# LANL-Bioinformatics/FaQCs

Hardware: AMD Instinct MI355X
Metric: M reads/sec (paired 2x150bp) (higher is better)
Workload: dtype u8; 1 GPU; synthetic 100M-pair 2x150bp Q33 reads resident in HBM per GPU, BWA_plus -q 5 --min_L 50, 1 step = 1 pass (trim_lds + counter all-reduce); pairs_per_gpu=100000000, read_len=150, terminal_n_supplied=True

## Files before the change

### faqcs_amd/csrc/faqcs_trim_common.h

```cpp
#pragma once
#include "faqcs_dev.h"

#include <stdlib.h>

static inline hipError_t ensure_dynamic_lds(const void *kernel, size_t bytes, unsigned long long &done)
{
    int dev = 0;
    hipError_t e = hipGetDevice(&dev);
    if (e != hipSuccess) return e;
    const unsigned long long bit = 1ull << (dev & 63);
    if (__atomic_load_n(&done, __ATOMIC_ACQUIRE) & bit) return hipSuccess;
    e = hipFuncSetAttribute(kernel, hipFuncAttributeMaxDynamicSharedMemorySize, (int)bytes);
    if (e == hipSuccess) __atomic_fetch_or(&done, bit, __ATOMIC_RELEASE);
    return e;
}

namespace {

template <int D> struct __attribute__((packed, aligned(1))) PackedBytes { uint32_t w[D]; };

__device__ __forceinline__ int med3i(int x, int lo, int hi) { return x < lo ? lo : (x > hi ? hi : x); }

template <int C> __device__ __forceinline__ uint32_t range_mask(int lo, int hi, int pbase)
{
// ... 246 lines not shown
    uint32_t *c = lane < FAQCS_NQ ? hrq + lane : hbq + (lane - FAQCS_NQ);
    if (in) { lds_add_u32_quiet(c, 1u); lds_add_u32_quiet(c, 1u); lds_add_u32_quiet(c, v); }
}
#endif

template <bool COMBINE = true>
__device__ __forceinline__ void chunk_epilogue_pre(const bool mine, const bool e_err, const uint32_t e_len, const int Vpre, const int lane, uint32_t *hlen,
                                                   uint32_t *hrq, uint32_t *hbqpre, const uint32_t *t_magic, FsAcc *defer)
{
        int qb_pre = 0;
        if (mine && e_len > 0 && Vpre > 0) qb_pre = e_len == 1 ? Vpre : (int)__umulhi((uint32_t)Vpre, t_magic[e_len]);
        qb_pre = qb_pre > 41 ? 41 : qb_pre;
        const bool act = mine && !e_err;
#ifdef FAQCS_LDS_DIAG_EPI_NOCONFLICT
        epi_diag_adds(act, e_len, hrq, hbqpre, lane);
#else
        const unsigned long long actm = COMBINE ? __ballot(act) : 0ull;
        if (!COMBINE) {
            if (act) {
                const uint32_t key = e_len | ((uint32_t)qb_pre << 16);
                const bool same = key == (uint32_t)__builtin_amdgcn_readfirstlane((int)key);
                const uint32_t cnt = (uint32_t)__builtin_popcountll(__ballot(same));
                if (same) {
                    if (lane == __ffsll((unsigned long long)__ballot(true)) - 1) {
                        lds_add_u32_quiet(hlen + e_len, cnt);
                        lds_add_u32_quiet(hrq + qb_pre, cnt);
                        if (e_len) lds_add_u32_quiet(hbqpre + qb_pre, cnt * e_len);
                    }
                } else {
                    lds_add_u32_quiet(hlen + e_len, 1u);
                    lds_add_u32_quiet(hrq + qb_pre, 1u);
                    if (e_len) lds_add_u32_quiet(hbqpre + qb_pre, e_len);
                }
            }
        } else if (actm != 0ull) {
            const uint32_t len0 = (uint32_t)__builtin_amdgcn_readlane((int)e_len, __builtin_ctzll(actm));
            const uint32_t cnt = wave_value_count(act, (uint32_t)qb_pre, lane);
            uint32_t bin = (uint32_t)lane;
            asm volatile("" : "+v"(bin));
            if (cnt) lds_add_u32_quiet(hrq + bin, cnt);
            len_hist_add(act, e_len, len0, 1u, hlen, lane);
            if (__ballot(act && e_len != len0) == 0ull) {
                if (cnt && len0) lds_add_u32_quiet(hbqpre + bin, cnt * len0);
            } else {
                peel_pairs(act && e_len != 0u, (uint32_t)qb_pre, e_len, nullptr, 0u, hbqpre, lane);
            }
        }
#endif
        const uint32_t one = 1u << 20;
        defer->tot += mine ? one | e_len : 0u;
}

template <int LPR>
__device__ __forceinline__ void chunk_epilogue(const ReadOutcome &o, const bool mine, const uint32_t my, const uint32_t v_len,
                                               const uint32_t v_hit, const int lane, uint32_t *hlen, uint32_t *hrq, uint32_t *hbqpre,
                                               uint32_t *hbqpost, uint32_t *lfs, const uint32_t *t_magic, uint2 *__restrict__ out,
                                               unsigned long long *__restrict__ rec_pre, unsigned long long *__restrict__ rec_post,
                                               const bool o_avgq_on, const uint32_t o_dbg, FsAcc *defer = nullptr, const bool wide_rt = false,
                                               const bool pre_done = false)
{
        const bool e_ret = (o.fl & FAQCS_F_VALID) != 0, e_err = (o.fl & FAQCS_F_ERR_QUALITY) != 0;
        const uint32_t e_len = v_len, e_n = o.an >> 16, e_filt = (o.fl & FAQCS_F_FILTER_MASK) >> FAQCS_F_FILTER_SHIFT;
        int qb_pre = 0, qb_post = 0;
        if (!defer && mine && e_len > 0 && o.Vpre > 0) qb_pre = e_len == 1 ? o.Vpre : (int)__umulhi((uint32_t)o.Vpre, t_magic[e_len]);
        if (e_ret && o.Vpost > 0) qb_post = e_n == 1 ? o.Vpost : (int)__umulhi((uint32_t)o.Vpost, t_magic[e_n]);
        qb_pre = qb_pre > 41 ? 41 : qb_pre;
        qb_post = qb_post > 41 ? 41 : qb_post;
        if (defer) {
            if (!pre_done) chunk_epilogue_pre<(LPR < 16)>(mine, e_err, e_len, o.Vpre, lane, hlen, hrq, hbqpre, t_magic, defer);
            const bool pact = mine && !e_err && e_ret;
#ifdef FAQCS_LDS_DIAG_EPI_NOCONFLICT
            epi_diag_adds(pact, e_n, hrq, hbqpost, lane);
#else
            const unsigned long long pm = LPR < 16 ? __ballot(pact) : 0ull;
            if (LPR >= 16) {
                if (pact) {
                    const uint32_t key = e_n | ((uint32_t)qb_post << 16);
                    const bool same = key == (uint32_t)__builtin_amdgcn_readfirstlane((int)key);
                    const uint32_t cnt = (uint32_t)__builtin_popcountll(__ballot(same));
                    if (same) {
                        if (lane == __ffsll((unsigned long long)__ballot(true)) - 1) {
                            lds_add_u32_quiet(hlen + e_n, cnt << 16);
                            lds_add_u32_quiet(hrq + qb_post, cnt << 16);
                            lds_add_u32_quiet(hbqpost + qb_post, cnt * e_n);
                        }
                    } else {
                        lds_add_u32_quiet(hlen + e_n, 0x10000u);
                        lds_add_u32_quiet(hrq + qb_post, 0x10000u);
                        lds_add_u32_quiet(hbqpost + qb_post, e_n);
                    }
                }
            } else if (pm != 0ull) {
                peel_pairs(pact, (uint32_t)qb_post, e_n, hrq, 0x10000u, hbqpost, lane);
                len_hist_add(pact, e_n, (uint32_t)__builtin_amdgcn_readlane((int)e_len, __builtin_ctzll(pm)), 0x10000u, hlen, lane);
            }
#endif
        } else if (!(o_dbg & 2u) && mine && !e_err) {
            atomicAdd(hlen + e_len, 1u);
            atomicAdd(hrq + qb_pre, 1u);
            if (e_len) atomicAdd(hbqpre + qb_pre, e_len);
            if (e_ret) {
                atomicAdd(hlen + e_n, 0x10000u);
                atomicAdd(hrq + qb_post, 0x10000u);
                atomicAdd(hbqpost + qb_post, e_n);
            }
        }
        if (mine) {
            const bool bad_base = v_hit == 0xffffu;
            out[my] = make_uint2(e_ret ? o.an : 0u, (o.fl & 0x3ffu) | (bad_base ? (uint32_t)FAQCS_F_ERR_BASE : (v_hit << 16)));
            const bool pre_on = !e_err, post_on = e_ret && !e_err;
            const unsigned long long pA = o.pAT & 0xffffu, pT = o.pAT >> 16, pC = o.pCG & 0xffffu, pG = o.pCG >> 16, pn = o.N & 0xffffu;
            const unsigned long long cA = o.cAT & 0xffffu, cT = o.cAT >> 16, cC = o.cCG & 0xffffu, cG = o.cCG >> 16, cn = o.N >> 16;
            if (LPR <= 16 && !wide_rt) {
                rec_pre[my] = pre_on ? (CR_VALID | e_len | (pA << 9) | (pT << 18) | (pC << 27) | (pG << 36) | (pn << 45)) : 0ull;
                rec_post[my] = post_on ? (CR_VALID | e_n | (cA << 9) | (cT << 18) | (cC << 27) | (cG << 36) | (cn << 45)) : 0ull;
            } else {
                reinterpret_cast<ulonglong2 *>(rec_pre)[my] =
                    pre_on ? make_ulonglong2(CR_VALID | e_len | (pA << 11) | (pT << 22) | (pC << 33), pG | (pn << 11)) : make_ulonglong2(0ull, 0ull);
                reinterpret_cast<ulonglong2 *>(rec_post)[my] =
                    post_on ? make_ulonglong2(CR_VALID | e_n | (cA << 11) | (cT << 22) | (cC << 33), cG | (cn << 11)) : make_ulonglong2(0ull, 0ull);
            }
        }
        const bool e_rlen = e_filt == FAQCS_FILT_LENGTH_PRE || e_filt == FAQCS_FILT_LENGTH_POST;
        const uint32_t one = 1u << 20;
        if (defer) {
            defer->trim += e_ret ? one | e_n : 0u;
            defer->len += e_rlen ? one | e_n : 0u;
            defer->qt += (o.fl & FAQCS_F_QUAL_TRIMMED) ? one | (o.fl >> 20) : 0u;
            const uint32_t m = one - 1u;
            const bool is_nn = (o.fl & FAQCS_F_POLY_N_SEEN) != 0, is_lc = e_filt == FAQCS_FILT_LOW_COMPLEXITY, is_avg = o_avgq_on && e_filt == FAQCS_FILT_AVG_Q;
            if (__any(is_nn)) { const uint32_t v = (uint32_t)wave_sum_i32((int)(is_nn ? one | e_n : 0u)); if (lane == 0) { lds_add_u32_quiet(&lfs[FAQCS_READ_NN], v >> 20); lds_add_u32_quiet(&lfs[FAQCS_BASE_NN], v & m); } }
            if (__any(is_lc)) { const uint32_t v = (uint32_t)wave_sum_i32((int)(is_lc ? one | e_n : 0u)); if (lane == 0) { lds_add_u32_quiet(&lfs[FAQCS_READ_LOW_COMPLEXITY], v >> 20); lds_add_u32_quiet(&lfs[FAQCS_BASE_LOW_COMPLEXITY], v & m); } }
            if (__any(is_avg)) { const uint32_t v = (uint32_t)wave_sum_i32((int)(is_avg ? one | e_n : 0u)); if (lane == 0) { lds_add_u32_quiet(&lfs[FAQCS_READ_AVG_Q], v >> 20); lds_add_u32_quiet(&lfs[FAQCS_BASE_AVG_Q], v & m); } }
            return;
        }
        const uint32_t s_tot = (uint32_t)wave_sum_i32((int)(mine ? one | e_len : 0u));
        const uint32_t s_trim = (uint32_t)wave_sum_i32((int)(e_ret ? one | e_n : 0u));
        const uint32_t s_len = (uint32_t)wave_sum_i32((int)(e_rlen ? one | e_n : 0u));
        const uint32_t s_nn = (uint32_t)wave_sum_i32((int)((o.fl & FAQCS_F_POLY_N_SEEN) ? one | e_n : 0u));
        const uint32_t s_qt = (uint32_t)wave_sum_i32((int)((o.fl & FAQCS_F_QUAL_TRIMMED) ? one | (o.fl >> 20) : 0u));
        const uint32_t s_lc = (uint32_t)wave_sum_i32((int)(e_filt == FAQCS_FILT_LOW_COMPLEXITY ? one | e_n : 0u));
        uint32_t s_avg = 0;
        if (o_avgq_on) s_avg = (uint32_t)wave_sum_i32((int)(e_filt == FAQCS_FILT_AVG_Q ? one | e_n : 0u));
        if (lane == 0) {
            const uint32_t m = one - 1u;
            if (s_tot) { atomicAdd(&lfs[FAQCS_TOTAL_COUNT], s_tot >> 20); atomicAdd(&lfs[FAQCS_TOTAL_NUMBER], s_tot >> 20); atomicAdd(&lfs[FAQCS_TOTAL_LENGTH], s_tot & m); }
            if (s_trim) { atomicAdd(&lfs[FAQCS_TOTAL_TRIMMED_NUMBER], s_trim >> 20); atomicAdd(&lfs[FAQCS_TOTAL_TRIMMED_LENGTH], s_trim & m); }
            if (s_len) { atomicAdd(&lfs[FAQCS_READ_LENGTH], s_len >> 20); atomicAdd(&lfs[FAQCS_BASE_LENGTH], s_len & m); }
            if (s_nn) { atomicAdd(&lfs[FAQCS_READ_NN], s_nn >> 20); atomicAdd(&lfs[FAQCS_BASE_NN], s_nn & m); }
            if (s_avg) { atomicAdd(&lfs[FAQCS_READ_AVG_Q], s_avg >> 20); atomicAdd(&lfs[FAQCS_BASE_AVG_Q], s_avg & m); }
            if (s_qt) { atomicAdd(&lfs[FAQCS_READ_QUAL_TRIM], s_qt >> 20); atomicAdd(&lfs[FAQCS_BASE_QUAL_TRIM], s_qt & m); }
            if (s_lc) { atomicAdd(&lfs[FAQCS_READ_LOW_COMPLEXITY], s_lc >> 20); atomicAdd(&lfs[FAQCS_BASE_LOW_COMPLEXITY], s_lc & m); }
        }
}

#ifdef __HIPCC__
__device__ __forceinline__ void comp_cell_add(uint32_t *tab, const uint32_t e, const uint32_t v, const int lane)
{
#ifdef FAQCS_DIAG_FOLD_NOCONFLICT
    constexpr uint32_t ND_ = (FAQCS_NCOMP_BIN * FAQCS_NCOMP_KIND + 1) / 2;
    uint32_t d = ((e >> 1) & ~63u) | (uint32_t)lane;
    d = d >= ND_ ? d - 64u : d;
    atomicAdd(&tab[d], v << (16 * (e & 1u)));
#else
    atomicAdd(&tab[e >> 1], v << (16 * (e & 1u)));
#endif
}
template <bool WIDE>
__device__ __forceinline__ void comp_fold_record(uint32_t *tab, const float *normt, const unsigned long long x, const unsigned long long y, const int lane)
{
    uint32_t nbin = 0xffffffffu;
    if (x & CR_VALID) {
        uint32_t len, cnt[5];
        if (WIDE) {
            len = (uint32_t)(x & 2047u);
// ... 97 lines not shown
```

### faqcs_amd/csrc/faqcs_trim_lds_kernel.hip

```cpp
#include "faqcs_trim_common.h"

#include <stdlib.h>
#include <type_traits>

#ifndef FAQCS_LDS_SUM_UNROLL
#define FAQCS_LDS_SUM_UNROLL 4
#endif
#ifndef FAQCS_LDS_SA_UNROLL
#define FAQCS_LDS_SA_UNROLL 2
#endif

namespace {

typedef uint32_t LdsPair2 __attribute__((ext_vector_type(2)));
typedef const __attribute__((address_space(3))) LdsPair2 *lds_u2c_ptr;
typedef __attribute__((address_space(3))) uint8_t *lds_u8_mut;
typedef const __attribute__((address_space(3))) uint8_t *lds_u8_ptr;
struct __attribute__((packed, aligned(1))) U32u { uint32_t w; };
typedef const __attribute__((address_space(3))) U32u *lds_u32u_ptr;

__device__ __forceinline__ uint32_t lds_ld(uint32_t byte_offset) { return *(lds_u32_ptr)(size_t)byte_offset; }
__device__ __forceinline__ uint32_t lds_ld_any(uint32_t byte_offset)
{
    const uint32_t a4 = byte_offset & ~3u;
// ... 601 lines not shown
                co += (uint32_t)__builtin_amdgcn_update_dpp(0, (int)co, 0x140, 0xf, 0xf, false);
            }
            tot_pe = turn ? pe : tot_pe; tot_po = turn ? po : tot_po; tot_ce = turn ? ce : tot_ce; tot_co = turn ? co : tot_co;
            if (WIDE) tot_pn = turn ? pn : tot_pn;
            }
            const uint32_t seam = e[C - 1].y & (uint32_t)__builtin_amdgcn_update_dpp(0, (int)e[0].y, 0x101, 0xf, 0xf, false) & 0x01000000u;
#ifdef FAQCS_LDS_DIAG_S_NO_NBLOCK
            const bool n_gate = false;
#else
            const bool n_gate = tq_lane + seam >= 0x02000000u || chk;
#endif
            if ((!EXT || P.max_poly_n == 2u) && __any(n_gate)) {
                uint32_t nb[D];
#pragma unroll
                for (int k = 0; k < D; ++k) {
                    const uint32_t orig = w[k] ^ (~((EXT && chk) ? 0u : inw[k]) & 0x88888888u);
                    const uint32_t x = (orig & inw[k]) ^ 0x4e4e4e4eu;
                    const uint32_t sx = (x & 0x7f7f7f7fu) + 0x7f7f7f7fu;
                    nb[k] = ~(sx | x) & 0x80808080u;
                }
                {
                    uint32_t hit = 0;
#pragma unroll
                    for (int k = 0; k < D; ++k) {
                        uint32_t here = nb[k];
                        if (4 * k + 4 > C) here &= low_bytes_(C - 4 * k);
                        const uint32_t next = k + 1 < D ? __builtin_amdgcn_alignbyte(nb[k + 1], nb[k], 1u) : (nb[k] >> 8);
                        hit |= here & next;
                    }
                    if (C % 4 == 0) hit |= (nb[D - 1] >> 24) & RW::next(nb[0] & 0x80u);
                    const bool rowhit = RW::all_or(hit) != 0u;
                    pairhit = turn ? rowhit : pairhit;
                }
            }
        }
    };
#define FAQCS_B_LOOP(I0, I1, CELLS)                                                                                   \
    {                                                                                                                 \
        _Pragma("unroll 1") for (int t = 0; t < TPR; ++t) {                                                          \
            if (base + (uint32_t)t >= n_reads) break;                       \
            const uint32_t a0_ = (uint32_t)__shfl((int)(I0), rowb + t), a1_ = (uint32_t)__shfl((int)(I1), rowb + t);   \
            RawB cur_;                                                                                                \
            load_b(a0_, a1_, cur_);                                                                                   \
            CELLS(cur_, a0_, a1_, t);                                                                                 \
        }                                                                                                             \
    }

#ifdef FAQCS_LDS_STAMPS
    unsigned long long st_acc[10] = {0, 0, 0, 0, 0, 0, 0, 0, 0, 0}, st_prev = 0, st_flush = 0, st_spill = 0;
#define FAQCS_STAMP(i) { const unsigned long long now_ = __builtin_amdgcn_s_memtime(); st_acc[i] += now_ - st_prev; st_prev = now_; }
#else
#define FAQCS_STAMP(i)
#endif
    uint32_t p_off = 0, p_end = 0, p_tn = 0;
    auto fetch_offsets = [&](const uint32_t chunk_) {
        if (chunk_ != NO_CHUNK) {
            const uint32_t lim_ = umin_(chunk_ * RPC + RPC, n_reads), my_ = owner ? chunk_ * RPC + ridx : lim_;
            p_off = off[my_ < lim_ ? my_ : lim_];
            p_end = off[my_ < lim_ ? my_ + 1 : lim_];
            if (tn_flags) p_tn = (uint32_t)tn_flags[my_ < lim_ ? my_ : lim_ - 1u];
        }
    };
    struct ChunkLoads { uint32_t v_off, v_end, v_sl, v_hit, pad_len, tn; };
    ChunkLoads ld = {0, 0, 0, 0, 0, 0};
    auto stage = [&](const uint8_t *arena, const uint32_t cs_, const uint32_t ce_, const uint32_t sh_, const uint32_t pad_len_) {
        if (pad_len_) dma_rows<NI>(arena + cs_ - sh_, pad_len_, (uint32_t)RPC, slot, lane);
        else dma_span<NI>(arena + cs_ - sh_, ce_ - cs_ + sh_, slot, lane);
    };
    bool pre_issued = false;
    auto issue_loads = [&](const uint32_t chunk_, const uint32_t o_, const uint32_t e_, const uint32_t tn_, ChunkLoads &L) {
        const uint32_t my_ = chunk_ * RPC + ridx;
        const bool mine_ = owner && my_ < n_reads;
        const uint32_t len_ = e_ - o_;
        const uint32_t cs_ = uniu(o_), ce_ = (uint32_t)__builtin_amdgcn_readlane((int)e_, 63);
        asm volatile("s_waitcnt lgkmcnt(0)" ::: "memory");
        const uint32_t shq_ = (uint32_t)((size_t)(qual + cs_) & 15u);
        const uint32_t len0_ = uniu(len_);
        const bool rows_ = (len0_ & 31u) == 0u && len0_ != 0u && len0_ <= (uint32_t)T::PADLEN && __all(!owner || (mine_ && len_ == len0_));
        L.pad_len = rows_ ? len0_ : 0u;
        stage(qual, cs_, ce_, shq_, L.pad_len);
        L.v_off = o_; L.v_end = e_; L.tn = tn_;
        L.v_sl = (WINDOWED && ad_sl && mine_) ? ad_sl[my_] : (len_ << 16);
        L.v_hit = (ad_hit && mine_) ? ad_hit[my_] : 0u;
    };
    uint32_t c_cur = (uint32_t)wave, n_flushed = 0, since_spill = 0;
    uint32_t chunk_cur = chunk_of(c_cur);
    fetch_offsets(chunk_cur);
#ifdef FAQCS_LDS_STAMPS
    const unsigned long long clk0 = __builtin_amdgcn_s_memtime(), rt0 = __builtin_amdgcn_s_memrealtime();
#endif
#pragma unroll 1
    for (;;) {
#ifdef FAQCS_LDS_STAMPS
        st_prev = __builtin_amdgcn_s_memtime();
#endif
        {
            const uint32_t n_local = lds_word(1);
            const uint32_t due = chunk_cur != NO_CHUNK ? c_cur / FLUSH_CHUNKS : (n_local + FLUSH_CHUNKS - 1) / FLUSH_CHUNKS;
#pragma unroll 1
            while (n_flushed < due) {
                spill_base_regs();
                flush_block_partial<C, LPR, NW>(smem, P.partials + ((size_t)blockIdx.x * FAQCS_PARTIAL_FLUSHES + n_flushed) * FAQCS_PARTIAL_ROW, tid);
                ++n_flushed; since_spill = 0;
            }
        }
#ifdef FAQCS_LDS_STAMPS
        st_flush += __builtin_amdgcn_s_memtime() - st_prev;
        st_prev = __builtin_amdgcn_s_memtime();
#endif
        if (chunk_cur == NO_CHUNK) break;
        uint32_t c_next = 0;
        if (lane == 0) c_next = __hip_atomic_fetch_add((lds_u32_mut)(size_t)(uint32_t)(T::O_CTR * 4), 1u, __ATOMIC_RELAXED, __HIP_MEMORY_SCOPE_WORKGROUP);
        c_next = uniu(c_next);
        const bool at_group_start = c_next % NW == 0 && c_next < lds_word(1);
        const bool fetch_group = at_group_start && c_next / NW + 1u < MAX_GROUPS;
        uint32_t g_new = 0;
        if (fetch_group && lane == 0) g_new = atomicAdd(g_next, 1u);
        const uint32_t chunk_next = chunk_of(c_next);
        {
            const uint32_t chunk = chunk_cur;
            const uint32_t base = chunk * RPC;
            const uint32_t my = base + ridx;
            const bool mine = owner && my < n_reads;
            if (!pre_issued) issue_loads(chunk_cur, p_off, p_end, p_tn, ld);
            const uint32_t v_off = ld.v_off, v_end = ld.v_end;
            const uint32_t v_len = v_end - v_off;
            const uint32_t v_sl = ld.v_sl, v_hit = ld.v_hit;
            const uint32_t cs = uniu(v_off), ce = (uint32_t)__builtin_amdgcn_readlane((int)v_end, 63);
            const int len = (int)v_len;
            const uint32_t shq = (uint32_t)((size_t)(qual + cs) & 15u);
            const uint32_t pad_len = uniu(ld.pad_len), pad_stride = pad_len + 16u;
            const uint32_t rowq = pad_len ? ridx * pad_stride + shq : v_off - cs + shq;
            const uint32_t span_q = pad_len ? (uint32_t)(RPC - 1) * pad_stride + pad_len + shq : ce - cs + shq;
            bool n_first = false, n_last = false;
            if (tn_flags) {
                const uint32_t f = mine ? ld.tn : 0u;
                n_first = (f & 1u) != 0u; n_last = (f & 2u) != 0u;
                fetch_offsets(chunk_next);
#ifdef FAQCS_LDS_DIAG_WAIT_ALL_AT_TOP
                asm volatile("s_waitcnt vmcnt(0)" ::: "memory");
#else
                if (chunk_next == NO_CHUNK) asm volatile("s_waitcnt vmcnt(0)" ::: "memory");
                else asm volatile("s_waitcnt vmcnt(3)" ::: "memory");
#endif
            } else {
                uint32_t bfirst = 0, blast = 0;
#ifndef FAQCS_LDS_NO_TERMINAL_LOADS
                if (len) { bfirst = (uint32_t)seq[(size_t)v_off]; blast = (uint32_t)seq[(size_t)v_off + len - 1]; }
#endif
                fetch_offsets(chunk_next);
                asm volatile("s_waitcnt vmcnt(0)" ::: "memory");
                asm volatile("" : "+v"(bfirst), "+v"(blast));
                n_first = bfirst == 'N'; n_last = blast == 'N';
            }
            if (at_group_start) {
                const uint32_t L1 = c_next / NW + 1u, gid = fetch_group ? gridDim.x + uniu(g_new) : n_groups;
                if (lane == 0) {
                    if (gid < n_groups) *(volatile __attribute__((address_space(3))) uint32_t *)(size_t)(uint32_t)((T::O_CTR + 4 + (int)(L1 & 3u)) * 4) = ((L1 & 0xfffu) << 20) | gid;
                    else *(volatile __attribute__((address_space(3))) uint32_t *)(size_t)(uint32_t)((T::O_CTR + 1) * 4) = L1 * NW;
                }
            }
            pad_behind_span<W, T::STG_BYTES>(slot_b, span_q, shq, lane, (uint32_t)in_off);
            FAQCS_STAMP(0)

            ReadOutcome oc;
            uint32_t v_patch = (uint32_t)len << 16;
            const bool tn = len > 0 && (n_first || n_last);
            if (__any(tn)) {
                int lead = 0, trail = len;
                bool go = tn && n_first;
#pragma unroll 1
                while (__any(go)) {
                    if (go) { ++lead; go = lead < len && seq[(size_t)v_off + lead] == 'N'; }
                }
                go = tn && n_last && lead < len;
                if (tn && lead >= len) trail = 0;
#pragma unroll 1
                while (__any(go)) {
                    if (go) { --trail; go = trail > 0 && seq[(size_t)v_off + trail - 1] == 'N'; }
                }
                if (tn) v_patch = (uint32_t)lead | ((uint32_t)trail << 16);
                const int ntail = tn ? len - trail : 0;
#pragma unroll 1
                for (int i = 0; __any(tn && (i < lead || i < ntail)); ++i) {
                    if (tn && i < lead) lds_st_u8(slot_b + rowq + (uint32_t)i, (uint32_t)in_off);
                    if (tn && i < ntail) lds_st_u8(slot_b + rowq + (uint32_t)(trail + i), (uint32_t)in_off);
                }
            }

            uint32_t qsum = 0, qacc = 0;
            int n_dw = 0;
            const uint32_t c_hi = 0x56565656u;
            bool sum_pass = !swar_ok || WINDOWED || (EXT && P.avgq_on);
            if (!sum_pass) {
                typedef uint32_t U4 __attribute__((ext_vector_type(4)));
                uint32_t acc = 0;
                const uint32_t n16 = (span_q + 15u) >> 4;
#pragma unroll
                for (int i = 0; i < NI; ++i) {
                    if ((uint32_t)(i * 64) >= n16) break;
                    if ((uint32_t)lane < n16 - (uint32_t)(i * 64)) {
                        const U4 v = *(const __attribute__((address_space(3))) U4 *)(size_t)((slot_b + (uint32_t)(lane * 16)) + (uint32_t)(i * 1024));
#pragma unroll
                        for (int e = 0; e < 4; ++e) { const uint32_t x = v[e] - offb; acc |= x | (x + c_hi) | v[e]; }
                    }
                }
                sum_pass = __any((acc & 0x80808080u) != 0u);
            }
            if (sum_pass) {
                const int nfull = len >> 2, rem = len & 3;
                const int kmax = uni((int)wave_max_u32((uint32_t)nfull));
                const uint32_t qa = slot_b + rowq, qa4 = qa & ~3u, qsh = qa & 3u;
                uint32_t prev = lds_ld(qa4);
#pragma unroll FAQCS_LDS_SUM_UNROLL
// ... 186 lines not shown
            int V_post = n * Q - ((wn * Q - V_win) - (S3 > 0 ? S3 : 0) - (S5 > 0 ? S5 : 0));
            if (EXT && sum_kept) {
                uint32_t sm = 0;
                const int k0 = a >> 2, k1 = (a + n + 3) >> 2;
                const int kmax = uni((int)wave_max_u32((uint32_t)(k1 > k0 ? k1 - k0 : 0)));
#pragma unroll 2
                for (int i = 0; i < kmax; ++i) {
                    const int k = k0 + i;
                    const uint32_t w = lds_ld_any(slot_b + rowq + 4u * (uint32_t)k);
                    const uint32_t m = low_bytes_(med3i(a + n - 4 * k, 0, 4)) & ~low_bytes_(med3i(a - 4 * k, 0, 4));
                    sm = __builtin_amdgcn_sad_u8(w & m, 0u, sm);
                }
                V_post = (int)sm - n * in_off;
            }
            if (__any(badq)) {
                const ExactQ xq = exact_quality(qual, v_off, len, v_patch, a, n, in_off, badq);
                if (badq) { V_pre = xq.sv; V_post = xq.svp; read_err = xq.mq > 41; }
            }
            const bool avgq_fail = EXT && P.avgq_on && V_post < ((const int32_t *)(smem + Cfg::O_TAVGQ))[n];

            FAQCS_STAMP(3)
            const uint32_t qi0 = rowq | ((uint32_t)len << 16);
            const bool retc = ret && !avgq_fail;
            const uint32_t qi1 = (uint32_t)a | ((uint32_t)n << AB) | (retc ? 1u << FB : 0u) | ((mine && !read_err) ? 1u << (FB + 1) : 0u);
#define FAQCS_QCELLS(X, A, B, T_) quality_cells(X, A, B, std::false_type{}, T_, !sum_pass)
            FAQCS_B_LOOP(qi0, qi1, FAQCS_QCELLS)
#undef FAQCS_QCELLS
            if (!sum_pass) {
                V_pre = (int)qb_sum - len * in_off;
                if (!(EXT && sum_kept)) V_post = n * Q - ((wn * Q - V_pre) - (S3 > 0 ? S3 : 0) - (S5 > 0 ? S5 : 0));
            }

            FAQCS_STAMP(4)
            asm volatile("s_waitcnt lgkmcnt(0)" ::: "memory");
            const uint32_t shs = (uint32_t)((size_t)(seq + cs) & 15u);
            stage(seq, cs, ce, shs, pad_len);
            const uint32_t rows = pad_len ? ridx * pad_stride + shs : v_off - cs + shs;
            FAQCS_STAMP(5)
#ifdef FAQCS_LDS_DIAG_NO_WORK_UNDER_DMA
            asm volatile("s_waitcnt vmcnt(0)" ::: "memory");
#endif
            chunk_epilogue_pre<(LPR < 16)>(mine, read_err, v_len, V_pre, lane, smem + Cfg::O_LEN, smem + Cfg::O_RQ, smem + Cfg::O_BQPRE, smem + Cfg::O_TMAGIC, &fs_acc);
            if (++since_spill == REG_FLUSH_EVERY) { spill_base_regs(); since_spill = 0; }
            const uint32_t si0 = rows | ((uint32_t)len << 16);
            const uint32_t si1 = (uint32_t)a | ((uint32_t)n << AB) | (retc ? 1u << FB : 0u) | ((mine && !read_err) ? 1u << (FB + 1) : 0u) |
                                 ((ret && !retc) ? 1u << (FB + 2) : 0u);
            const uint32_t vpk = WIDE ? (uint32_t)V_pre : (((uint32_t)V_pre & 0xffffu) | ((uint32_t)V_post << 16)), vpk2 = WIDE ? (uint32_t)V_post : 0u;
            const uint32_t fpk = flags | (filt << FAQCS_F_FILTER_SHIFT);
            const uint32_t v_hit_w = v_hit;
#ifdef FAQCS_LDS_STAMPS
            { const unsigned long long now_ = __builtin_amdgcn_s_memtime(); st_spill += now_ - st_prev; st_prev = now_; }
#endif
            asm volatile("s_waitcnt vmcnt(0) lgkmcnt(0)" ::: "memory");
            asm volatile("" : "+v"(p_off), "+v"(p_end), "+v"(p_tn));
            any_err |= p_tn << 1;
            FAQCS_STAMP(5)

#define FAQCS_S_BODY(I1, MODE)                                                                                        \
            if (base + (uint32_t)t >= n_reads) break;                       \
            const uint32_t a1_ = (uint32_t)__shfl((int)(I1), rowb + t);                                               \
            if (MODE == 1 && !__any(((a1_ >> FB) & 1u) != 0u)) continue;                                              \
            const uint32_t a0_ = (uint32_t)__shfl((int)si0, rowb + t);                                                \
            base_step(t, a0_, a1_, std::integral_constant<int, MODE>{});
#define FAQCS_S_LOOP(I1, MODE, FLAT)                                                                                  \
    {                                                                                                                 \
        int t = 0;                                                                                                    \
        if (MODE == 0) pairhit = false;                                                                               \
        if constexpr (FLAT && SCATTER) {                                                                              \
            _Pragma("unroll") for (; t < TPR; ++t) { FAQCS_S_BODY(I1, MODE) }                                         \
        } else {                                                                                                      \
            _Pragma("unroll 1") for (; t < TPR; ++t) { FAQCS_S_BODY(I1, MODE) }                                       \
        }                                                                                                             \
        if (MODE == 0) totals_finish(t);                                                                              \
    }
            seen7 = 0;
            FAQCS_S_LOOP(si1, 0, true)
            if (__any((seen7 & 0x80808080u) != 0u)) {
                FAQCS_S_LOOP(si1, 2, false)
                asm volatile("s_waitcnt lgkmcnt(0)" ::: "memory");
#pragma unroll 1
                for (int p = 0; __any(p < len); ++p) {
                    if (p < len && (lds_ld_u8(slot_b + rows + (uint32_t)p) & 0x80u)) lds_st_u8(slot_b + rows + (uint32_t)p, 0u);
                }
                asm volatile("s_waitcnt lgkmcnt(0)" ::: "memory");
                FAQCS_S_LOOP(si1, 0, false)
            }

            FAQCS_STAMP(6)
            {
            const int len = (int)(si0 >> 16), a = (int)(si1 & AM), n = (int)((si1 >> AB) & AM);
            const uint32_t rows = si0 & 0xffffu, rowq = rows - shs + shq, v_off = pad_len ? cs + ridx * pad_len : cs + rows - shs, v_len = (uint32_t)len;
            const uint32_t qi0 = rowq | ((uint32_t)len << 16);
            int V_pre = WIDE ? (int)vpk : (int)(int16_t)(uint16_t)(vpk & 0xffffu), V_post = WIDE ? (int)vpk2 : (int)vpk >> 16;
            uint32_t flags = fpk & ~(uint32_t)FAQCS_F_FILTER_MASK, filt = (fpk & (uint32_t)FAQCS_F_FILTER_MASK) >> FAQCS_F_FILTER_SHIFT;
            const uint32_t v_hit = WINDOWED ? v_hit_w : 0u;
            uint32_t pA = tot_pe & 0xfffu, pC = (tot_pe >> 12) & 0xfffu, pN = WIDE ? tot_pn & 0xffffu : tot_pe >> 24, pT = tot_po & 0xfffu, pG = tot_po >> 12;
            uint32_t cA = tot_ce & 0xfffu, cC = (tot_ce >> 12) & 0xfffu, cN = WIDE ? tot_pn >> 16 : tot_ce >> 24, cT = tot_co & 0xfffu, cG = tot_co >> 12;
            {
                bool polyn;
                if (EXT && P.max_poly_n != 2u) {
                    uint32_t run[NWORD], hit = 0, nub[NWORD];
#pragma unroll
                    for (int wd = 0; wd < NWORD; ++wd) nub[wd] = 0;
                    const bool scan = P.max_poly_n != 0u && ret && (cN >= P.max_poly_n || !retc);
                    if (__any(scan)) {
                        const int kmax = uni((int)wave_max_u32(scan ? (uint32_t)((len + 3) >> 2) : 0u));
#pragma unroll
// ... 87 lines not shown

            FAQCS_STAMP(7)
            const bool veto = retc && !ret;
            if (__any(veto)) {
                const uint32_t vi1 = (uint32_t)a | ((uint32_t)n << AB) | (veto ? 1u << FB : 0u) | (veto ? 1u << (FB + 1) : 0u);
                FAQCS_S_LOOP(vi1, 1, false)
                asm volatile("s_waitcnt lgkmcnt(0)" ::: "memory");
                stage(qual, cs, ce, shq, pad_len);
                asm volatile("s_waitcnt vmcnt(0)" ::: "memory");
#ifdef FAQCS_LDS_DIAG_VERIFY_RESTAGE
                if (!pad_len) {
                    const uint32_t nb_ = ce - cs + shq;
                    uint32_t bad_ = 0, first_ = 0xffffffffu;
                    for (uint32_t u_ = (uint32_t)lane; u_ * 16u < nb_; u_ += 64u) {
                        const uint4 g_ = *reinterpret_cast<const uint4 *>(qual + cs - shq + (size_t)u_ * 16u);
                        const uint32_t l0_ = lds_ld(slot_b + u_ * 16u), l1_ = lds_ld(slot_b + u_ * 16u + 4u), l2_ = lds_ld(slot_b + u_ * 16u + 8u), l3_ = lds_ld(slot_b + u_ * 16u + 12u);
                        if (g_.x != l0_ || g_.y != l1_ || g_.z != l2_ || g_.w != l3_) { ++bad_; first_ = first_ == 0xffffffffu ? u_ : first_; }
                    }
                    if (bad_) {
                        atomicAdd(reinterpret_cast<unsigned long long *>(err + 16), (unsigned long long)bad_);
                        atomicMax(reinterpret_cast<unsigned long long *>(err + 16) + 1, ((unsigned long long)nb_ << 32) | first_);
                    }
                    atomicAdd(reinterpret_cast<unsigned long long *>(err + 16) + 2, 1ull);
                }
#endif
                pad_behind_span<W, T::STG_BYTES>(slot_b, pad_len ? (uint32_t)(RPC - 1) * pad_stride + pad_len + shq : ce - cs + shq, shq, lane, (uint32_t)in_off);
                if (__any((veto && tn) || badq)) {
#pragma unroll 1
                    for (int p = 0; __any(((veto && tn) || badq) && p < len); ++p) {
                        if (((veto && tn) || badq) && p < len) {
                            const uint32_t r = lds_ld_u8(slot_b + rowq + (uint32_t)p);
                            int v = (int)(int8_t)r - in_off;
                            v = v < 0 ? 0 : (v > 41 ? 41 : v);
                            if (p < (int)(v_patch & 0xffffu) || p >= (int)(v_patch >> 16)) v = 0;
                            lds_st_u8(slot_b + rowq + (uint32_t)p, (uint32_t)(v + in_off));
                        }
                    }
                }
                const uint32_t ui1 = (uint32_t)a | ((uint32_t)n << AB) | (veto ? 1u << FB : 0u);
#pragma unroll 1
                for (int t = 0; t < TPR; ++t) {
                    const uint32_t i1 = (uint32_t)__shfl((int)ui1, rowb + t);
                    if (!__any(((i1 >> FB) & 1u) != 0u)) continue;
                    const uint32_t i0 = (uint32_t)__shfl((int)qi0, rowb + t);
                    RawB x;
                    load_b(i0, i1, x);
                    quality_cells(x, i0, i1, std::true_type{}, t, false);
                }
                asm volatile("s_waitcnt lgkmcnt(0)" ::: "memory");
            }
#undef FAQCS_S_LOOP
#undef FAQCS_S_BODY

            ChunkLoads ld_next = ld;
            pre_issued = chunk_next != NO_CHUNK;
            if (pre_issued) issue_loads(chunk_next, p_off, p_end, any_err >> 1, ld_next);
            any_err &= 1u;

            if (read_err) { any_err = 1; flags |= FAQCS_F_ERR_QUALITY; }
            oc.an = (uint32_t)a | ((uint32_t)n << 16);
            oc.fl = flags | (ret ? FAQCS_F_VALID : 0u) | (filt << FAQCS_F_FILTER_SHIFT);
            oc.pAT = pA | (pT << 16); oc.pCG = pC | (pG << 16);
            oc.cAT = cA | (cT << 16); oc.cCG = cC | (cG << 16);
            oc.N = pN | (cN << 16);
            oc.Vpre = V_pre; oc.Vpost = V_post;

            chunk_epilogue<LPR>(oc, mine, my, v_len, v_hit, lane, smem + Cfg::O_LEN, smem + Cfg::O_RQ, smem + Cfg::O_BQPRE,
                                smem + Cfg::O_BQPOST, smem + Cfg::O_FS, smem + Cfg::O_TMAGIC, out, rec_pre, rec_post, EXT && P.avgq_on != 0, 0u, &fs_acc,
                                WIDE && P.wide_records != 0u, true);
            ld = ld_next;
            }
        }

        FAQCS_STAMP(8)
        c_cur = c_next; chunk_cur = chunk_next;
    }
    if (__any((any_err & 1u) != 0) && lane == 0) atomicOr(err, 1u);
    if (tid == 0) P.partial_rows[blockIdx.x] = n_flushed;
    if (lds_tail_folds_v<C, NW, LPR, RPC> && P.fold_n) {
        __syncthreads();
        comp_fold_tail<NW * 64>(smem, P, tid, blockIdx.x & 1u);
    }
#ifdef FAQCS_LDS_STAMPS
    if (lane == 0) {
#pragma unroll
        for (int i = 0; i < 9; ++i) atomicAdd(reinterpret_cast<unsigned long long *>(err + 16) + i, st_acc[i]);
        atomicAdd(reinterpret_cast<unsigned long long *>(err + 16) + 9, __builtin_amdgcn_s_memtime() - clk0);
        atomicAdd(reinterpret_cast<unsigned long long *>(err + 16) + 11, st_flush);
#ifdef FAQCS_LDS_BLOCKLOG
        if (wave == 0) printf("block %u xcc %u chunks %u start %llu end %llu\n", blockIdx.x, __builtin_amdgcn_s_getreg((20 << 0) | (0 << 6) | (3 << 11)), smem[T::O_CTR + 1],
                              (unsigned long long)rt0, (unsigned long long)__builtin_amdgcn_s_memrealtime());
#endif
        if (wave == 0) {
            const unsigned long long te = __builtin_amdgcn_s_memrealtime();
            atomicMax(reinterpret_cast<unsigned long long *>(err + 16) + 13, te);
            atomicMax(reinterpret_cast<unsigned long long *>(err + 16) + 14, ~te);
            atomicMax(reinterpret_cast<unsigned long long *>(err + 16) + 15, ~rt0);
        }
        atomicAdd(reinterpret_cast<unsigned long long *>(err + 16) + 12, st_spill);
        (void)clk_entry;
        atomicAdd(reinterpret_cast<unsigned long long *>(err + 16) + 10, __builtin_amdgcn_s_memrealtime() - rt0);
    }
#endif
#undef FAQCS_STAMP
}

__global__ __launch_bounds__(256) void terminal_n_flags(const uint8_t *__restrict__ seq, const uint32_t *__restrict__ off, const uint32_t n, uint8_t *__restrict__ flags)
{
    const uint32_t i = blockIdx.x * 256u + threadIdx.x;
    if (i >= n) return;
    const uint32_t a = off[i], b = off[i + 1];
    flags[i] = b > a ? (uint8_t)((seq[a] == 'N' ? 1u : 0u) | (seq[(size_t)b - 1] == 'N' ? 2u : 0u)) : (uint8_t)0;
}
hipError_t faqcs_launch_terminal_n_flags(const uint8_t *seq, const uint32_t *off, uint32_t n_reads, uint8_t *flags, hipStream_t st)
{
    if (!n_reads) return hipSuccess;
    hipLaunchKernelGGL(terminal_n_flags, dim3((n_reads + 255) / 256), dim3(256), 0, st, seq, off, n_reads, flags);
    return hipGetLastError();
}

template <int C, bool WINDOWED, bool EXT, int LPR = 8, int RPC = 64>
static hipError_t launch_trim_lds(const TrimPlan &plan, const DevParams &P, const TrimArgs &a)
{
    constexpr int NW = lds_waves(C, LPR, RPC);
    constexpr size_t lds = (size_t)LdsCfg<C, NW, LPR, RPC>::lds_dwords() * 4;
    static unsigned long long attr_done = 0;
    auto kern = trim_lds<C, NW, WINDOWED, EXT, LPR, RPC>;
    if (plan.NW != NW || plan.RPC != RPC) return hipErrorInvalidValue;
    if (hipError_t e = ensure_dynamic_lds(reinterpret_cast<const void *>(kern), lds, attr_done); e != hipSuccess) return e;
    if (plan.grid == 0) return hipSuccess;
    hipLaunchKernelGGL(kern, dim3(plan.grid), dim3(NW * 64), lds, a.st, P, a.seq, a.qual, a.off, a.n_reads, a.ad_sl, a.ad_hit,
                       reinterpret_cast<uint2 *>(a.out), a.rec_pre, a.rec_post, a.counters, a.err, a.tn_flags);
    if (hipError_t e = hipGetLastError(); e != hipSuccess) return e;
    hipLaunchKernelGGL((fold_partials<C, LPR>), dim3((RowCfg<C, LPR, lds_wq(C, LPR)>::N_ZERO + 63) / 64), dim3(1024), 0, a.st, P.partials, P.partial_rows, plan.grid, a.counters, P.lay, a.err + 8);
    return hipGetLastError();
}

using TrimLaunch = hipError_t (*)(const TrimPlan &, const DevParams &, const TrimArgs &);
template <int C, int LPR, int RPC> static TrimLaunch trim_lds_variant(const TrimPlan &plan)
{
    return plan.ext ? (plan.windowed ? launch_trim_lds<C, true, true, LPR, RPC> : launch_trim_lds<C, false, true, LPR, RPC>)
                    : (plan.windowed ? launch_trim_lds<C, true, false, LPR, RPC> : launch_trim_lds<C, false, false, LPR, RPC>);
}

hipError_t faqcs_launch_trim_lds(const TrimPlan &plan, const DevParams &P, const TrimArgs &a)
{
    TrimLaunch f = nullptr;
    switch (trim_shape_key(plan.C, plan.LPR)) {
    case trim_shape_key(13, 4): f = trim_lds_variant<13, 4, 64>(plan); break;
    case trim_shape_key(19, 4): f = trim_lds_variant<19, 4, 64>(plan); break;
    case trim_shape_key(13, 8): f = trim_lds_variant<13, 8, 64>(plan); break;
// ... 7 lines not shown
```

Before: 9371 M reads/s.

## Issue output stores before next-chunk prefetch and defer group-claim atomic publish

Per-read output and record stores are split out of the epilogue and now issue before the next chunk's loads, so they no longer queue behind the prefetch. The global group-claim atomic moves from the loop top to after the terminal-N wait, and its result is published to LDS only after the later vmcnt(0) drain. This keeps the atomic's latency off the top-of-loop wait. Several diagnostic ifdef variants and a top-wait timing stamp are added, and the atomic changes from atomicAdd to atomicInc.

```diff
diff --git a/faqcs_amd/csrc/faqcs_trim_common.h b/faqcs_amd/csrc/faqcs_trim_common.h
--- a/faqcs_amd/csrc/faqcs_trim_common.h
+++ b/faqcs_amd/csrc/faqcs_trim_common.h
@@ -322,12 +322,37 @@
 }
 
 template <int LPR>
+__device__ __forceinline__ void chunk_outputs(const ReadOutcome &o, const bool mine, const uint32_t my, const uint32_t v_len, const uint32_t v_hit,
+                                              uint2 *__restrict__ out, unsigned long long *__restrict__ rec_pre,
+                                              unsigned long long *__restrict__ rec_post, const bool wide_rt)
+{
+        const bool e_ret = (o.fl & FAQCS_F_VALID) != 0, e_err = (o.fl & FAQCS_F_ERR_QUALITY) != 0;
+        const uint32_t e_len = v_len, e_n = o.an >> 16;
+        if (mine) {
+            const bool bad_base = v_hit == 0xffffu;
+            out[my] = make_uint2(e_ret ? o.an : 0u, (o.fl & 0x3ffu) | (bad_base ? (uint32_t)FAQCS_F_ERR_BASE : (v_hit << 16)));
+            const bool pre_on = !e_err, post_on = e_ret && !e_err;
+            const unsigned long long pA = o.pAT & 0xffffu, pT = o.pAT >> 16, pC = o.pCG & 0xffffu, pG = o.pCG >> 16, pn = o.N & 0xffffu;
+            const unsigned long long cA = o.cAT & 0xffffu, cT = o.cAT >> 16, cC = o.cCG & 0xffffu, cG = o.cCG >> 16, cn = o.N >> 16;
+            if (LPR <= 16 && !wide_rt) {
+                rec_pre[my] = pre_on ? (CR_VALID | e_len | (pA << 9) | (pT << 18) | (pC << 27) | (pG << 36) | (pn << 45)) : 0ull;
+                rec_post[my] = post_on ? (CR_VALID | e_n | (cA << 9) | (cT << 18) | (cC << 27) | (cG << 36) | (cn << 45)) : 0ull;
+            } else {
+                reinterpret_cast<ulonglong2 *>(rec_pre)[my] =
+                    pre_on ? make_ulonglong2(CR_VALID | e_len | (pA << 11) | (pT << 22) | (pC << 33), pG | (pn << 11)) : make_ulonglong2(0ull, 0ull);
+                reinterpret_cast<ulonglong2 *>(rec_post)[my] =
+                    post_on ? make_ulonglong2(CR_VALID | e_n | (cA << 11) | (cT << 22) | (cC << 33), cG | (cn << 11)) : make_ulonglong2(0ull, 0ull);
+            }
+        }
+}
+
+template <int LPR>
 __device__ __forceinline__ void chunk_epilogue(const ReadOutcome &o, const bool mine, const uint32_t my, const uint32_t v_len,
                                                const uint32_t v_hit, const int lane, uint32_t *hlen, uint32_t *hrq, uint32_t *hbqpre,
                                                uint32_t *hbqpost, uint32_t *lfs, const uint32_t *t_magic, uint2 *__restrict__ out,
                                                unsigned long long *__restrict__ rec_pre, unsigned long long *__restrict__ rec_post,
                                                const bool o_avgq_on, const uint32_t o_dbg, FsAcc *defer = nullptr, const bool wide_rt = false,
-                                               const bool pre_done = false)
+                                               const bool pre_done = false, const bool stores_done = false)
 {
         const bool e_ret = (o.fl & FAQCS_F_VALID) != 0, e_err = (o.fl & FAQCS_F_ERR_QUALITY) != 0;
         const uint32_t e_len = v_len, e_n = o.an >> 16, e_filt = (o.fl & FAQCS_F_FILTER_MASK) >> FAQCS_F_FILTER_SHIFT;
@@ -375,22 +400,7 @@
                 atomicAdd(hbqpost + qb_post, e_n);
             }
         }
-        if (mine) {
-            const bool bad_base = v_hit == 0xffffu;
-            out[my] = make_uint2(e_ret ? o.an : 0u, (o.fl & 0x3ffu) | (bad_base ? (uint32_t)FAQCS_F_ERR_BASE : (v_hit << 16)));
-            const bool pre_on = !e_err, post_on = e_ret && !e_err;
-            const unsigned long long pA = o.pAT & 0xffffu, pT = o.pAT >> 16, pC = o.pCG & 0xffffu, pG = o.pCG >> 16, pn = o.N & 0xffffu;
-            const unsigned long long cA = o.cAT & 0xffffu, cT = o.cAT >> 16, cC = o.cCG & 0xffffu, cG = o.cCG >> 16, cn = o.N >> 16;
-            if (LPR <= 16 && !wide_rt) {
-                rec_pre[my] = pre_on ? (CR_VALID | e_len | (pA << 9) | (pT << 18) | (pC << 27) | (pG << 36) | (pn << 45)) : 0ull;
-                rec_post[my] = post_on ? (CR_VALID | e_n | (cA << 9) | (cT << 18) | (cC << 27) | (cG << 36) | (cn << 45)) : 0ull;
-            } else {
-                reinterpret_cast<ulonglong2 *>(rec_pre)[my] =
-                    pre_on ? make_ulonglong2(CR_VALID | e_len | (pA << 11) | (pT << 22) | (pC << 33), pG | (pn << 11)) : make_ulonglong2(0ull, 0ull);
-                reinterpret_cast<ulonglong2 *>(rec_post)[my] =
-                    post_on ? make_ulonglong2(CR_VALID | e_n | (cA << 11) | (cT << 22) | (cC << 33), cG | (cn << 11)) : make_ulonglong2(0ull, 0ull);
-            }
-        }
+        if (!stores_done) chunk_outputs<LPR>(o, mine, my, v_len, v_hit, out, rec_pre, rec_post, wide_rt);
         const bool e_rlen = e_filt == FAQCS_FILT_LENGTH_PRE || e_filt == FAQCS_FILT_LENGTH_POST;
         const uint32_t one = 1u << 20;
         if (defer) {
diff --git a/faqcs_amd/csrc/faqcs_trim_lds_kernel.hip b/faqcs_amd/csrc/faqcs_trim_lds_kernel.hip
--- a/faqcs_amd/csrc/faqcs_trim_lds_kernel.hip
+++ b/faqcs_amd/csrc/faqcs_trim_lds_kernel.hip
@@ -677,6 +677,14 @@
 #else
 #define FAQCS_STAMP(i)
 #endif
+#if defined(FAQCS_LDS_STAMPS) && defined(FAQCS_LDS_DIAG_STAMP_TOP_WAIT)
+    unsigned long long st_topwait = 0, st_tw0 = 0;
+#define FAQCS_TOP_WAIT_BEGIN asm volatile("s_memtime %0\n\ts_waitcnt lgkmcnt(0)" : "=s"(st_tw0) : : "memory");
+#define FAQCS_TOP_WAIT_END { unsigned long long tw1_; asm volatile("s_memtime %0\n\ts_waitcnt lgkmcnt(0)" : "=s"(tw1_) : : "memory"); st_topwait += tw1_ - st_tw0; }
+#else
+#define FAQCS_TOP_WAIT_BEGIN
+#define FAQCS_TOP_WAIT_END
+#endif
     uint32_t p_off = 0, p_end = 0, p_tn = 0;
     auto fetch_offsets = [&](const uint32_t chunk_) {
         if (chunk_ != NO_CHUNK) {
@@ -693,6 +701,10 @@
         else dma_span<NI>(arena + cs_ - sh_, ce_ - cs_ + sh_, slot, lane);
     };
     bool pre_issued = false;
+#ifdef FAQCS_LDS_DIAG_STALE_STORES
+    ReadOutcome oc_prev = {0, 0, 0, 0, 0, 0, 0, 0, 0};
+    uint32_t v_len_prev = 0, v_hit_prev = 0;
+#endif
     auto issue_loads = [&](const uint32_t chunk_, const uint32_t o_, const uint32_t e_, const uint32_t tn_, ChunkLoads &L) {
         const uint32_t my_ = chunk_ * RPC + ridx;
         const bool mine_ = owner && my_ < n_reads;
@@ -737,11 +749,17 @@
         uint32_t c_next = 0;
         if (lane == 0) c_next = __hip_atomic_fetch_add((lds_u32_mut)(size_t)(uint32_t)(T::O_CTR * 4), 1u, __ATOMIC_RELAXED, __HIP_MEMORY_SCOPE_WORKGROUP);
         c_next = uniu(c_next);
+        uint32_t g_new = 0;
+#ifdef FAQCS_LDS_DIAG_EARLY_CLAIM
         const bool at_group_start = c_next % NW == 0 && c_next < lds_word(1);
         const bool fetch_group = at_group_start && c_next / NW + 1u < MAX_GROUPS;
-        uint32_t g_new = 0;
         if (fetch_group && lane == 0) g_new = atomicAdd(g_next, 1u);
         const uint32_t chunk_next = chunk_of(c_next);
+#else
+        const uint32_t chunk_next = chunk_of(c_next);
+        const bool at_group_start = c_next % NW == 0 && chunk_next != NO_CHUNK;
+        const bool fetch_group = at_group_start && c_next / NW + 1u < MAX_GROUPS;
+#endif
         {
             const uint32_t chunk = chunk_cur;
             const uint32_t base = chunk * RPC;
@@ -762,29 +780,40 @@
                 const uint32_t f = mine ? ld.tn : 0u;
                 n_first = (f & 1u) != 0u; n_last = (f & 2u) != 0u;
                 fetch_offsets(chunk_next);
+                FAQCS_TOP_WAIT_BEGIN
 #ifdef FAQCS_LDS_DIAG_WAIT_ALL_AT_TOP
                 asm volatile("s_waitcnt vmcnt(0)" ::: "memory");
 #else
                 if (chunk_next == NO_CHUNK) asm volatile("s_waitcnt vmcnt(0)" ::: "memory");
                 else asm volatile("s_waitcnt vmcnt(3)" ::: "memory");
 #endif
+                FAQCS_TOP_WAIT_END
             } else {
                 uint32_t bfirst = 0, blast = 0;
 #ifndef FAQCS_LDS_NO_TERMINAL_LOADS
                 if (len) { bfirst = (uint32_t)seq[(size_t)v_off]; blast = (uint32_t)seq[(size_t)v_off + len - 1]; }
 #endif
                 fetch_offsets(chunk_next);
+                FAQCS_TOP_WAIT_BEGIN
                 asm volatile("s_waitcnt vmcnt(0)" ::: "memory");
+                FAQCS_TOP_WAIT_END
                 asm volatile("" : "+v"(bfirst), "+v"(blast));
                 n_first = bfirst == 'N'; n_last = blast == 'N';
             }
-            if (at_group_start) {
-                const uint32_t L1 = c_next / NW + 1u, gid = fetch_group ? gridDim.x + uniu(g_new) : n_groups;
-                if (lane == 0) {
-                    if (gid < n_groups) *(volatile __attribute__((address_space(3))) uint32_t *)(size_t)(uint32_t)((T::O_CTR + 4 + (int)(L1 & 3u)) * 4) = ((L1 & 0xfffu) << 20) | gid;
-                    else *(volatile __attribute__((address_space(3))) uint32_t *)(size_t)(uint32_t)((T::O_CTR + 1) * 4) = L1 * NW;
-                }
-            }
+            auto publish_group = [&]() {
+                if (at_group_start) {
+                    const uint32_t L1 = c_next / NW + 1u, gid = fetch_group ? gridDim.x + uniu(g_new) : n_groups;
+                    if (lane == 0) {
+                        if (gid < n_groups) *(volatile __attribute__((address_space(3))) uint32_t *)(size_t)(uint32_t)((T::O_CTR + 4 + (int)(L1 & 3u)) * 4) = ((L1 & 0xfffu) << 20) | gid;
+                        else *(volatile __attribute__((address_space(3))) uint32_t *)(size_t)(uint32_t)((T::O_CTR + 1) * 4) = L1 * NW;
+                    }
+                }
+            };
+#ifdef FAQCS_LDS_DIAG_EARLY_CLAIM
+            publish_group();
+#else
+            if (fetch_group && lane == 0) g_new = atomicInc(g_next, 0xffffffffu);
+#endif
             pad_behind_span<W, T::STG_BYTES>(slot_b, span_q, shq, lane, (uint32_t)in_off);
             FAQCS_STAMP(0)
 
@@ -1077,7 +1106,10 @@
             { const unsigned long long now_ = __builtin_amdgcn_s_memtime(); st_spill += now_ - st_prev; st_prev = now_; }
 #endif
             asm volatile("s_waitcnt vmcnt(0) lgkmcnt(0)" ::: "memory");
-            asm volatile("" : "+v"(p_off), "+v"(p_end), "+v"(p_tn));
+            asm volatile("" : "+v"(p_off), "+v"(p_end), "+v"(p_tn), "+v"(g_new));
+#ifndef FAQCS_LDS_DIAG_EARLY_CLAIM
+            publish_group();
+#endif
             any_err |= p_tn << 1;
             FAQCS_STAMP(5)
 
@@ -1271,22 +1303,45 @@
 #undef FAQCS_S_LOOP
 #undef FAQCS_S_BODY
 
-            ChunkLoads ld_next = ld;
-            pre_issued = chunk_next != NO_CHUNK;
-            if (pre_issued) issue_loads(chunk_next, p_off, p_end, any_err >> 1, ld_next);
-            any_err &= 1u;
-
-            if (read_err) { any_err = 1; flags |= FAQCS_F_ERR_QUALITY; }
+            if (read_err) flags |= FAQCS_F_ERR_QUALITY;
             oc.an = (uint32_t)a | ((uint32_t)n << 16);
             oc.fl = flags | (ret ? FAQCS_F_VALID : 0u) | (filt << FAQCS_F_FILTER_SHIFT);
             oc.pAT = pA | (pT << 16); oc.pCG = pC | (pG << 16);
             oc.cAT = cA | (cT << 16); oc.cCG = cC | (cG << 16);
             oc.N = pN | (cN << 16);
             oc.Vpre = V_pre; oc.Vpost = V_post;
-
+            const bool wide_rt = WIDE && P.wide_records != 0u;
+#if defined(FAQCS_LDS_DIAG_STALE_STORES)
+            {
+                const ReadOutcome oc_st = pre_issued ? oc_prev : oc;
+                chunk_outputs<LPR>(oc_st, mine, my, pre_issued ? v_len_prev : v_len, pre_issued ? v_hit_prev : v_hit, out, rec_pre, rec_post, wide_rt);
+                oc_prev = oc; v_len_prev = v_len; v_hit_prev = v_hit;
+            }
+#elif !defined(FAQCS_LDS_DIAG_LATE_STORES)
+            chunk_outputs<LPR>(oc, mine, my, v_len, v_hit, out, rec_pre, rec_post, wide_rt);
+#endif
+
+            ChunkLoads ld_next = ld;
+#ifdef FAQCS_LDS_DIAG_NO_EARLY_QDMA
+            pre_issued = false;
+#else
+            pre_issued = chunk_next != NO_CHUNK;
+#endif
+            if (pre_issued) issue_loads(chunk_next, p_off, p_end, any_err >> 1, ld_next);
+#ifdef FAQCS_LDS_DIAG_NO_EARLY_QDMA
+            p_tn = any_err >> 1;
+#endif
+            any_err &= 1u;
+            if (read_err) any_err = 1;
+
+#ifdef FAQCS_LDS_DIAG_LATE_STORES
+            constexpr bool stores_done = false;
+#else
+            constexpr bool stores_done = true;
+#endif
             chunk_epilogue<LPR>(oc, mine, my, v_len, v_hit, lane, smem + Cfg::O_LEN, smem + Cfg::O_RQ, smem + Cfg::O_BQPRE,
                                 smem + Cfg::O_BQPOST, smem + Cfg::O_FS, smem + Cfg::O_TMAGIC, out, rec_pre, rec_post, EXT && P.avgq_on != 0, 0u, &fs_acc,
-                                WIDE && P.wide_records != 0u, true);
+                                wide_rt, true, stores_done);
             ld = ld_next;
             }
         }
@@ -1314,8 +1369,13 @@
             const unsigned long long te = __builtin_amdgcn_s_memrealtime();
             atomicMax(reinterpret_cast<unsigned long long *>(err + 16) + 13, te);
             atomicMax(reinterpret_cast<unsigned long long *>(err + 16) + 14, ~te);
+#ifndef FAQCS_LDS_DIAG_STAMP_TOP_WAIT
             atomicMax(reinterpret_cast<unsigned long long *>(err + 16) + 15, ~rt0);
-        }
+#endif
+        }
+#ifdef FAQCS_LDS_DIAG_STAMP_TOP_WAIT
+        atomicAdd(reinterpret_cast<unsigned long long *>(err + 16) + 15, st_topwait);
+#endif
         atomicAdd(reinterpret_cast<unsigned long long *>(err + 16) + 12, st_spill);
         (void)clk_entry;
         atomicAdd(reinterpret_cast<unsigned long long *>(err + 16) + 10, __builtin_amdgcn_s_memrealtime() - rt0);
```

After: 9455 M reads/s (median of 6 runs). About the same (+0.9%).
